# Chriz122/ultralytics_pro

Hardware: AMD Instinct MI355X
Metric: images/sec (whole job = n_gpus x per-GPU bs=32) YOLOv8n 640x640 (forward + Detect decode + NMS) (higher is better)
Workload: dtype bf16

## Files before the change

include/upa.h:

```cpp
#ifndef UPA_H
#define UPA_H
#include <stddef.h>
#include <stdint.h>

#ifdef __cplusplus
extern "C" {
#endif

enum { UPA_F32 = 0, UPA_BF16 = 1, UPA_U8_BGR_HWC = 2  };
enum { UPA_ACT_NONE = 0, UPA_ACT_SILU = 1, UPA_ACT_RELU = 2 };
enum { UPA_OK = 0, UPA_EINVAL = -1, UPA_EUNSUPPORTED = -2, UPA_EWORKSPACE = -3, UPA_ELAUNCH = -4 };

typedef struct upa_opts {
  uint32_t size;
  int32_t conv_big;
  int32_t conv_big_bm;
  int32_t conv_ckt;
  int32_t no_ws, no_pipe, no_1x1, no_c16, no_upcat;
  int32_t pipe_all;
  int32_t pipe_min_tiles;
  int32_t pipe_wgs, c16_wgs;
  int32_t c1_mt, c1_waves, c1_wgs;
  int32_t pair;
  int32_t pair_tile64, pair_tile32;
// ... 2 lines not shown
  int32_t c2f16_waves;
  int32_t c2f32_th;
  int32_t no_branch_tail;
  int32_t branch_tail_bm;
  int32_t stem_wgs, stemf_wgs, stemf_waves, stem_no_mfma;
  int32_t ablate_conv, ablate_pipe, ablate_c1, ablate_stem;
  int32_t c2f64_max_px;
  int32_t conv_ws3;
  int32_t no_group;
  int32_t no_c2f32_up;
  int32_t no_xcd;
  int32_t keys_only;
  int32_t conv_p8;
  int32_t c2f_stream;
  int32_t c2f_stream_rows;
  int32_t no_stack_first;
  int32_t no_epi_stats;
  int32_t nms_stages;
  int32_t nms_first_prefix;
  int32_t detect_stream;
  int32_t detect_stream_rows;
  int32_t no_sppf_front;
  int32_t no_c2f16_down;
} upa_opts;

int upa_version(void);
const char* upa_last_error(void);
size_t upa_opts_size(void);

size_t upa_conv_packed_weight_bytes(int cout, int cin, int k, int dtype);
int upa_pack_conv_weight(const float* w_oihw, int cout, int cin, int k, int dtype, void* out);
int upa_conv2d_bias_act(const void* x, int n, int h, int w, int cin, int ldx,
                        const void* w_packed, const float* bias ,
                        void* y, int cout, int ldy,
                        const void* residual , int ldr,
                        int k, int stride, int pad, int act, int dtype, const upa_opts* opts, void* stream);
typedef struct upa_conv_problem {
  const void* x; int32_t n, h, w, cin, ldx;
  const void* w_packed; const float* bias;
  void* y; int32_t cout, ldy;
  const void* residual; int32_t ldr;
} upa_conv_problem;
int upa_conv2d_bias_act_group(const upa_conv_problem* probs, int count, int k, int stride, int pad, int act, int dtype,
                              const upa_opts* opts, void* stream);

int upa_conv2d_pool2(const void* x, int n, int h, int w, int cin, int ldx, const void* w_packed, const float* bias, void* y, int cout,
// ... 358 lines not shown
```

ultralytics_pro_amd/_lib.py:

```python

from __future__ import annotations

import ctypes as C
import os
from pathlib import Path

import torch

UPA_F32, UPA_BF16, UPA_U8_BGR_HWC = 0, 1, 2
UPA_EINVAL = -1
UPA_EUNSUPPORTED = -2
ACT_NONE, ACT_SILU, ACT_RELU = 0, 1, 2
UPA_PAD_GATHER, UPA_PAD_SCATTER_COPY, UPA_PAD_SCATTER_ADD = 1, 2, 4
MASKS_PLANES, MASKS_OVERLAP = 0, 1
MASK_U8, MASK_F32, MASK_I32 = 0, 1, 2

_PKG = Path(__file__).resolve().parent
LIB_PATH = Path(os.environ.get("UPA_HIP_LIB", _PKG / "libupa_hip.so"))

_vp, _i, _f, _sz = C.c_void_p, C.c_int, C.c_float, C.c_size_t


class Opts(C.Structure):

    _fields_ = [("size", C.c_uint32), ("conv_big", _i), ("conv_big_bm", _i), ("conv_ckt", _i),
                ("no_ws", _i), ("no_pipe", _i), ("no_1x1", _i), ("no_c16", _i), ("no_upcat", _i),
                ("pipe_all", _i), ("pipe_min_tiles", _i), ("pipe_wgs", _i), ("c16_wgs", _i),
                ("c1_mt", _i), ("c1_waves", _i), ("c1_wgs", _i),
                ("pair", _i), ("pair_tile64", _i), ("pair_tile32", _i), ("no_pair_cv2", _i),
                ("c2f", _i), ("c2f16_waves", _i), ("c2f32_th", _i),
                ("no_branch_tail", _i), ("branch_tail_bm", _i),
                ("stem_wgs", _i), ("stemf_wgs", _i), ("stemf_waves", _i), ("stem_no_mfma", _i),
                ("ablate_conv", _i), ("ablate_pipe", _i), ("ablate_c1", _i), ("ablate_stem", _i), ("c2f64_max_px", _i), ("conv_ws3", _i), ("no_group", _i), ("no_c2f32_up", _i), ("no_xcd", _i), ("keys_only", _i), ("conv_p8", _i), ("c2f_stream", _i), ("c2f_stream_rows", _i), ("no_stack_first", _i), ("no_epi_stats", _i), ("nms_stages", _i), ("nms_first_prefix", _i), ("detect_stream", _i), ("detect_stream_rows", _i), ("no_sppf_front", _i), ("no_c2f16_down", _i)]

    def __init__(self, **kw):
        super().__init__()
        self.size = C.sizeof(Opts)
        for k, v in kw.items():
            if k in dict(self._fields_):
                setattr(self, k, int(v))
            else:
                raise AttributeError(f"upa_opts has no field '{k}'")

    def replace(self, **kw) -> "Opts":
        o = Opts()
        C.memmove(C.byref(o), C.byref(self), C.sizeof(Opts))
        for k, v in kw.items():
            setattr(o, k, int(v))
        return o

    _ENV = {"UPA_CONV_BIG": ("conv_big", lambda v: {0: 1, 1: 0, 2: 2}[int(v)]), "UPA_CONV_BIG_BM": ("conv_big_bm", int), "UPA_CONV_WS3": ("conv_ws3", int),
            "UPA_CONV_CKT": ("conv_ckt", int), "UPA_CONV_NO_WS": ("no_ws", lambda v: 1), "UPA_CONV_NO_PIPE": ("no_pipe", lambda v: 1),
            "UPA_CONV_NO_1X1": ("no_1x1", lambda v: 1), "UPA_CONV_NO_C16": ("no_c16", lambda v: 1), "UPA_NO_UPCAT": ("no_upcat", lambda v: 1),
            "UPA_PIPE_ALL": ("pipe_all", lambda v: 1), "UPA_PIPE_MIN_TILES": ("pipe_min_tiles", int), "UPA_PIPE_WGS": ("pipe_wgs", int),
            "UPA_C16_WGS": ("c16_wgs", int), "UPA_C1_MT": ("c1_mt", int), "UPA_C1_WAVES": ("c1_waves", int), "UPA_C1_WGS": ("c1_wgs", int),
            "UPA_NO_PAIR": ("pair", lambda v: {0: 2, 1: 1, 2: 0, 3: 3}[int(v)]), "UPA_PAIR_T64": ("pair_tile64", int),
# ... 245 lines not shown
```

ultralytics_pro_amd/csrc/conv_big.hip:

```cpp
#include <stdlib.h>

#include <mutex>
#include <type_traits>
#include <unordered_map>

#include "common.h"
#include "conv_pipe.h"
UPA_STAMP_DEFINE(conv_big)

template <int KS, int STRIDE, int WM, int WN, int MT, int NT, int TAIL = 0>
__device__ __forceinline__ void conv_big_body(const BigParams& p, const int bid0) {
  static_assert(WM * WN == 8, "8 waves per workgroup");
  static_assert(TAIL == 0 || TAIL == 3 || TAIL == 4 || WN == 1, "a tail needs every channel of a pixel in one wave");
  static_assert(TAIL != 1 || (NT % 2) == 0, "box branch: 64 channels");
  static_assert(TAIL != 3 || (NT % 2) == 0, "the statistics epilogue pairs n-tiles");
  static_assert(TAIL != 4 || ((NT % 2) == 0 && KS == 2 && STRIDE == 1), "the interleaving epilogue: 2 x 2 phase kernels, paired n-tiles");
  constexpr int NTB = WN * NT;
  constexpr int WBUF = 2 * NTB * 1024;
  extern __shared__ __attribute__((aligned(16))) char smem[];
  const int tid = threadIdx.x;
  const int lane = tid & 63;
  const int wave = __builtin_amdgcn_readfirstlane(tid >> 6);
  const int r = lane & 15, g = lane >> 4;
  const int wm = wave / WN, wn = wave % WN;

  const int tilesPerImg = p.tilesX * p.tilesY;
  int bid = p.no_xcd ? bid0 : upa_xcd_tile(bid0, tilesPerImg * p.N);
  const int n = bid / tilesPerImg;
  bid -= n * tilesPerImg;
  const int tyi = bid / p.tilesX;
  const int txi = bid - tyi * p.tilesX;
  const int oy0 = tyi * p.TH, ox0 = txi * p.TW;
  const int iy0 = oy0 * STRIDE - p.pad, ix0 = ox0 * STRIDE - p.pad;
  const int ntb0 = blockIdx.y * NTB;

  const int haloItems = p.IH * p.IWp * 8;
  const int haloPadded = (haloItems + 63) & ~63;
  char* hal = smem;
  char* wbuf = smem + (size_t)haloPadded * 16;

  int pl0[MT], pty[MT], ptx[MT];
#pragma unroll
  for (int i = 0; i < MT; ++i) {
    const int pp = (wm * MT + i) * 16 + r;
    int ty = (int)__umulhi((unsigned)pp, p.magicTW);
    int tx = pp - ty * p.TW;
    if (ty >= p.TH) { ty = p.TH; tx = 0; }
    pty[i] = ty;
    ptx[i] = tx;
    pl0[i] = ty < p.TH ? (ty * STRIDE) * p.IWp + tx : 0;
  }

  f32x4 acc[MT][NT];
#pragma unroll
  for (int i = 0; i < MT; ++i)
#pragma unroll
    for (int j = 0; j < NT; ++j) acc[i][j] = f32x4{0.f, 0.f, 0.f, 0.f};

  constexpr int TAPS = KS * KS;
  const int nChunks = (p.KTT + 1) >> 1;

  auto stage_halo = [&](int c) __attribute__((always_inline)) {
    const int c0 = c * 64;
    for (int base = wave * 64; base < haloPadded; base += 512) {
      const int idx = base + lane;
      const int pix = idx >> 3;
      const int slot = idx & 7;
      const int cg = slot ^ (pix & 7);
      const int py = (int)__umulhi((unsigned)pix, p.magicIW);
      const int qx = pix - py * p.IWp;
      int px = qx;
      if constexpr (STRIDE == 2) px = qx < p.HALF ? 2 * qx : 2 * (qx - p.HALF) + 1;
      const int iy = iy0 + py, ix = ix0 + px;
      const int ch = c0 + cg * 8;
      const char* src = reinterpret_cast<const char*>(g_zero16);
      if (idx < haloItems && px < p.IW && iy >= 0 && iy < p.H && ix >= 0 && ix < p.W && ch < p.Cin)
        src = p.x + ((((size_t)n * p.H + iy) * p.W + ix) * (size_t)p.ldx + ch) * 2;
      lds_dma16(src, hal + base * 16);
    }
  };
  auto stage_w = [&](int c, int tap, int b) __attribute__((always_inline)) {
#pragma unroll
    for (int f0 = 0; f0 < 2 * NTB; f0 += 8) {
      const int f = f0 + wave;
      if (f < 2 * NTB) {
        const int kt = f / NTB, j = f - kt * NTB;
        const int ktg = c * 2 + kt;
        const int nt = ntb0 + j;
        const char* src = reinterpret_cast<const char*>(g_zero16);
        if (ktg < p.KTT && nt < p.NTn) src = p.w + (((size_t)(tap * p.KTT + ktg) * p.NTn + nt) * 64 + lane) * 16;
        lds_dma16(src, wbuf + b * WBUF + f * 1024);
      }
    }
  };

  UPA_STAMP_AT(0);
  UPA_STAMP_HWID();
  stage_halo(0);
  stage_w(0, 0, 0);
  int buf = 0;
  for (int c = 0; c < nChunks; ++c) {
    int kh = 0, kw = 0;
#pragma unroll 1
    for (int tap = 0; tap < TAPS; ++tap) {
      asm volatile("s_waitcnt vmcnt(0)" ::: "memory");
      __syncthreads();
      if (c == 0) UPA_STAMP_AT(1 + tap);
      if (tap + 1 < TAPS) stage_w(c, tap + 1, buf ^ 1);
      const int tapshift = kh * p.IWp + (STRIDE == 2 ? (kw >> 1) + (kw & 1) * p.HALF : kw);
      const char* wb = wbuf + buf * WBUF + (wn * NT) * 1024 + lane * 16;
      int paddr[MT], pswz[MT];
#pragma unroll
      for (int i = 0; i < MT; ++i) {
        const int pl = pl0[i] + tapshift;
        paddr[i] = pl * 128;
        pswz[i] = pl & 7;
      }
#pragma unroll
      for (int kt = 0; kt < 2; ++kt) {
        if constexpr (TAIL == 2) {
          if (kt == 1 && c * 2 + 1 >= p.KTT) break;
        }
        if constexpr (NT <= 6) {
          u32x4 a[NT], b[MT];
#pragma unroll
          for (int j = 0; j < NT; ++j) a[j] = *reinterpret_cast<const u32x4*>(wb + (kt * NTB + j) * 1024);
#pragma unroll
          for (int i = 0; i < MT; ++i) b[i] = *reinterpret_cast<const u32x4*>(hal + paddr[i] + (((kt * 4 + g) ^ pswz[i]) << 4));
#pragma unroll
          for (int i = 0; i < MT; ++i)
#pragma unroll
            for (int j = 0; j < NT; ++j)
              acc[i][j] = __builtin_amdgcn_mfma_f32_16x16x32_bf16(*reinterpret_cast<const bf16x8*>(&a[j]),
                                                                  *reinterpret_cast<const bf16x8*>(&b[i]), acc[i][j], 0, 0, 0);
        } else {
          constexpr int GS = (NT + 1) / 2;
          u32x4 b[MT];
#pragma unroll
          for (int i = 0; i < MT; ++i) b[i] = *reinterpret_cast<const u32x4*>(hal + paddr[i] + (((kt * 4 + g) ^ pswz[i]) << 4));
#pragma unroll
          for (int j0 = 0; j0 < NT; j0 += GS) {
            u32x4 a[GS];
#pragma unroll
            for (int j = 0; j < GS; ++j)
              if (j0 + j < NT) a[j] = *reinterpret_cast<const u32x4*>(wb + (kt * NTB + j0 + j) * 1024);
#pragma unroll
            for (int i = 0; i < MT; ++i)
#pragma unroll
              for (int j = 0; j < GS; ++j)
                if (j0 + j < NT)
                  acc[i][j0 + j] = __builtin_amdgcn_mfma_f32_16x16x32_bf16(*reinterpret_cast<const bf16x8*>(&a[j]),
                                                                           *reinterpret_cast<const bf16x8*>(&b[i]), acc[i][j0 + j], 0, 0, 0);
            __builtin_amdgcn_sched_barrier(0);
          }
        }
      }
      buf ^= 1;
      if (++kw == KS) { kw = 0; ++kh; }
    }
    if (c + 1 < nChunks) {
      __syncthreads();
      stage_halo(c + 1);
      stage_w(c + 1, 0, buf);
    }
  }
  UPA_STAMP_AT(10);

  if constexpr (TAIL == 1 || TAIL == 2) {
    f32x4 bv[NT];
#pragma unroll
    for (int j = 0; j < NT; ++j) bv[j] = *reinterpret_cast<const f32x4*>(p.bias + j * 16 + g * 4);
    f32x4 acc2[MT][NT];
#pragma unroll
    for (int i = 0; i < MT; ++i)
#pragma unroll
      for (int j = 0; j < NT; ++j) acc2[i][j] = f32x4{0.f, 0.f, 0.f, 0.f};
#pragma unroll
    for (int s2 = 0; s2 < NT / 2; ++s2) {
      u32x4 hb[MT];
#pragma unroll
      for (int i = 0; i < MT; ++i) {
        float v0[4], v1[4];
#pragma unroll
        for (int q = 0; q < 4; ++q) {
          v0[q] = act_rcp<UPA_ACT_SILU>(acc[i][2 * s2][q] + bv[2 * s2][q]);
          v1[q] = act_rcp<UPA_ACT_SILU>(acc[i][2 * s2 + 1][q] + bv[2 * s2 + 1][q]);
// ... 201 lines not shown
            const u32x2 rv = *reinterpret_cast<const u32x2*>(rrow + cb * 2);
            v[0] += __uint_as_float(rv[0] << 16); v[1] += __uint_as_float(rv[0] & 0xFFFF0000u);
            v[2] += __uint_as_float(rv[1] << 16); v[3] += __uint_as_float(rv[1] & 0xFFFF0000u);
          }
          *reinterpret_cast<u32x2*>(yrow + cb * 2) = u32x2{pack_bf16x2(v[0], v[1]), pack_bf16x2(v[2], v[3])};
        }
      }
    }
  };
  if (p.act == UPA_ACT_SILU) epilogue(std::integral_constant<int, UPA_ACT_SILU>{});
  else if (p.act == UPA_ACT_RELU) epilogue(std::integral_constant<int, UPA_ACT_RELU>{});
  else epilogue(std::integral_constant<int, UPA_ACT_NONE>{});
  UPA_STAMP_AT(11);
#ifdef UPA_STAMP
  asm volatile("s_waitcnt vmcnt(0)" ::: "memory");
  UPA_STAMP_AT(12);
#endif
}

template <int KS, int STRIDE, int WM, int WN, int MT, int NT, int TAIL = 0>
__global__ __launch_bounds__(512, 4) void conv_big_kernel(const BigParams p) {
  conv_big_body<KS, STRIDE, WM, WN, MT, NT, TAIL>(p, (int)blockIdx.x);
}

template <int KS, int STRIDE, int WM, int WN, int MT, int NT, int TAIL = 0>
__global__ __launch_bounds__(512, 4) void conv_big_pair_kernel(const BigParams p0, const BigParams p1, const int split) {
  if ((int)blockIdx.x < split) conv_big_body<KS, STRIDE, WM, WN, MT, NT, TAIL>(p0, (int)blockIdx.x);
  else conv_big_body<KS, STRIDE, WM, WN, MT, NT, TAIL>(p1, (int)blockIdx.x - split);
}
template <int KS, int STRIDE, int WM, int WN, int MT, int NT, int TAIL = 0>
__global__ __launch_bounds__(512, 4) void conv_big_tri_kernel(const BigParams p0, const BigParams p1, const BigParams p2, const int s0,
                                                              const int s1) {
  if ((int)blockIdx.x < s0) conv_big_body<KS, STRIDE, WM, WN, MT, NT, TAIL>(p0, (int)blockIdx.x);
  else if ((int)blockIdx.x < s1) conv_big_body<KS, STRIDE, WM, WN, MT, NT, TAIL>(p1, (int)blockIdx.x - s0);
  else conv_big_body<KS, STRIDE, WM, WN, MT, NT, TAIL>(p2, (int)blockIdx.x - s1);
}

template <int KS_, int STRIDE_, int WM_, int WN_, int MT_, int NT_, int TAIL_>
struct BigCfg {
  static constexpr int NTB = WN_ * NT_;
  __device__ static __forceinline__ void run(const BigParams& p, int bid) { conv_big_body<KS_, STRIDE_, WM_, WN_, MT_, NT_, TAIL_>(p, bid); }
};
template <class CA, class CB>
__global__ __launch_bounds__(512, 4) void conv_big_mix_kernel(const BigParams a0, const BigParams a1, const BigParams b0, const BigParams b1,
                                                              const int s0, const int s1, const int s2) {
  const int b = (int)blockIdx.x;
  if (b < s0) CA::run(a0, b);
  else if (b < s1) CA::run(a1, b - s0);
  else if (b < s2) CB::run(b0, b - s1);
  else CB::run(b1, b - s2);
}

namespace {
void big_halo_geometry(BigParams& p, bool tight = false) {
  p.IH = (p.TH - 1) * p.stride + p.KS;
  p.IW = (p.TW - 1) * p.stride + p.KS;
  p.HALF = p.stride == 2 ? (p.IW + 1) / 2 : 0;
  const int minp = p.stride == 2 ? 2 * p.HALF : p.IW;
  p.IWp = tight ? minp : upa_lds_pick_pitch(minp, p.TW, p.TH * p.TW, p.stride);
  p.magicTW = (unsigned)((0x100000000ULL + p.TW - 1) / p.TW);
  p.magicIW = (unsigned)((0x100000000ULL + p.IWp - 1) / p.IWp);
}
size_t big_halo_bytes(const BigParams& p) { return (((size_t)p.IH * p.IWp * 8 + 63) & ~(size_t)63) * 16; }

bool big_pick_tile(BigParams& p, int bm, int ntb, size_t lds_cap) {
  struct Pick { int th, tw, tight; };
  static std::mutex mu;
  static std::unordered_map<unsigned long long, Pick> memo;
  const unsigned long long key = ((unsigned long long)p.OH << 48) ^ ((unsigned long long)p.OW << 32) ^ ((unsigned long long)bm << 20) ^
                                 ((unsigned long long)ntb << 12) ^ ((unsigned long long)(lds_cap >> 9) << 3) ^ ((unsigned long long)p.KS << 56) ^ (p.KS == 3 ? 4u : 0u) ^
                                 (p.stride == 2 ? 2u : 0u);
  {
    std::lock_guard<std::mutex> lk(mu);
// ... 21 lines not shown
        big_halo_geometry(p, tight != 0);
        const size_t lds = big_halo_bytes(p) + 2 * (size_t)(2 * ntb * 1024) + 256;
        if (lds > lds_cap) continue;
        const long tiles = (long)cdiv(p.OW, tw) * cdiv(p.OH, th);
        const long cost = tiles * 65536 + (long)p.IH * p.IWp;
        if (best < 0 || cost < best) { best = cost; bth = th; btw = tw; btight = tight != 0; }
        break;
      }
    }
  }
  p.TH = bth; p.TW = btw;
  if (best >= 0) big_halo_geometry(p, btight);
  {
    std::lock_guard<std::mutex> lk(mu);
    memo[key] = Pick{best >= 0 ? bth : 0, btw, btight ? 1 : 0};
  }
  return best >= 0;
}

template <int KS, int STRIDE, int WM, int WN, int MT, int NT, int TAIL = 0>
int big_launch_inst(const BigParams& p, size_t lds, hipStream_t s) {
  constexpr int NTB = WN * NT;
  const dim3 grid((unsigned)((long)p.tilesX * p.tilesY * p.N), (unsigned)cdiv(p.NTn, NTB));
  auto kern = conv_big_kernel<KS, STRIDE, WM, WN, MT, NT, TAIL>;
  if (hipError_t e = upa_full_lds<conv_big_kernel<KS, STRIDE, WM, WN, MT, NT, TAIL>>(); e != hipSuccess) {
    upa_set_error("conv_big: cannot raise LDS limit: %s", hipGetErrorString(e));
    return UPA_ELAUNCH;
  }
  hipLaunchKernelGGL(kern, grid, dim3(512), lds, s, p);
  UPA_LAUNCH_CHECK();
  return UPA_OK;
}

template <int KS, int STRIDE, int WM, int WN, int MT, int NT, int TAIL = 0>
int big_launch_pair_inst(const BigParams& p0, const BigParams& p1, size_t lds, hipStream_t s) {
  constexpr int NTB = WN * NT;
  const long t0 = (long)p0.tilesX * p0.tilesY * p0.N, t1 = (long)p1.tilesX * p1.tilesY * p1.N;
  if (cdiv(p0.NTn, NTB) != cdiv(p1.NTn, NTB) || t0 + t1 >= (1L << 31)) return UPA_EUNSUPPORTED;
  const dim3 grid((unsigned)(t0 + t1), (unsigned)cdiv(p0.NTn, NTB));
  if (hipError_t e = upa_full_lds<conv_big_pair_kernel<KS, STRIDE, WM, WN, MT, NT, TAIL>>(); e != hipSuccess) {
    upa_set_error("conv_big: cannot raise LDS limit: %s", hipGetErrorString(e));
    return UPA_ELAUNCH;
  }
  hipLaunchKernelGGL((conv_big_pair_kernel<KS, STRIDE, WM, WN, MT, NT, TAIL>), grid, dim3(512), lds, s, p0, p1, (int)t0);
  UPA_LAUNCH_CHECK();
  return UPA_OK;
}

template <int KS, int STRIDE, int WM, int WN, int MT, int NT, int TAIL = 0>
int big_launch_tri_inst(const BigParams& p0, const BigParams& p1, const BigParams& p2, size_t lds, hipStream_t s) {
  constexpr int NTB = WN * NT;
  const long t0 = (long)p0.tilesX * p0.tilesY * p0.N, t1 = (long)p1.tilesX * p1.tilesY * p1.N, t2 = (long)p2.tilesX * p2.tilesY * p2.N;
  if (cdiv(p0.NTn, NTB) != cdiv(p1.NTn, NTB) || cdiv(p0.NTn, NTB) != cdiv(p2.NTn, NTB) || t0 + t1 + t2 >= (1L << 31)) return UPA_EUNSUPPORTED;
  const dim3 grid((unsigned)(t0 + t1 + t2), (unsigned)cdiv(p0.NTn, NTB));
  if (hipError_t e = upa_full_lds<conv_big_tri_kernel<KS, STRIDE, WM, WN, MT, NT, TAIL>>(); e != hipSuccess) {
    upa_set_error("conv_big: cannot raise LDS limit: %s", hipGetErrorString(e));
    return UPA_ELAUNCH;
  }
  hipLaunchKernelGGL((conv_big_tri_kernel<KS, STRIDE, WM, WN, MT, NT, TAIL>), grid, dim3(512), lds, s, p0, p1, p2, (int)t0, (int)(t0 + t1));
  UPA_LAUNCH_CHECK();
  return UPA_OK;
}

template <class CA, class CB>
int big_launch_mix(const BigParams* pa, int na, const BigParams* pb, int nb, size_t lds, hipStream_t s) {
  long t[4] = {0, 0, 0, 0};
  for (int i = 0; i < na; ++i) { t[i] = (long)pa[i].tilesX * pa[i].tilesY * pa[i].N; if (pa[i].NTn > CA::NTB) return UPA_EUNSUPPORTED; }
  for (int i = 0; i < nb; ++i) { t[2 + i] = (long)pb[i].tilesX * pb[i].tilesY * pb[i].N; if (pb[i].NTn > CB::NTB) return UPA_EUNSUPPORTED; }
  const long tot = t[0] + t[1] + t[2] + t[3];
  if (tot >= (1L << 31)) return UPA_EUNSUPPORTED;
  if (hipError_t e = upa_full_lds<conv_big_mix_kernel<CA, CB>>(); e != hipSuccess) {
    upa_set_error("conv_big: cannot raise LDS limit: %s", hipGetErrorString(e));
    return UPA_ELAUNCH;
  }
  hipLaunchKernelGGL((conv_big_mix_kernel<CA, CB>), dim3((unsigned)tot), dim3(512), lds, s, pa[0], pa[na > 1 ? 1 : 0], pb[0], pb[nb > 1 ? 1 : 0],
                     (int)t[0], (int)(t[0] + t[1]), (int)(t[0] + t[1] + t[2]));
  UPA_LAUNCH_CHECK();
  return UPA_OK;
}

template <int WM, int WN, int MT, int NT>
int big_launch_ks(const BigParams& p, size_t lds, hipStream_t s) {
  if (p.KS == 1) return big_launch_inst<1, 1, WM, WN, MT, NT>(p, lds, s);
  if (p.KS == 2) return big_launch_inst<2, 1, WM, WN, MT, NT>(p, lds, s);
  if (p.stride == 2) return big_launch_inst<3, 2, WM, WN, MT, NT>(p, lds, s);
  return big_launch_inst<3, 1, WM, WN, MT, NT>(p, lds, s);
}
}

extern "C" size_t upa_tail_packed_weight_bytes(int cout, int cin) {
  return (size_t)cdiv(cin, 32) * cdiv(cout, 16) * 1024;
}

// ... 207 lines not shown
  p.NTn = (p.Cout + 15) / 16;
  ntb = p.NTn <= 4 ? 4 : (p.NTn <= 6 ? 6 : 8);
  if (p.NTn == 5 && p.KS == 3 && p.stride == 1) ntb = 5;
  if (p.NTn == 9 && p.KS == 3 && p.stride == 1) ntb = 9;
  if (force_ntb == 5 && p.NTn <= 5 && p.KS == 3 && p.stride == 1) ntb = 5;
  const long px = (long)p.N * p.OH * p.OW;
  if (ntb == 8 && p.NTn % 4 == 0 && (px + 127) / 128 * cdiv(p.NTn, 8) < upa_num_cus()) ntb = 4;
  const int cols = cdiv(p.NTn, ntb);
  bm = 256;
  if ((px + 255) / 256 * cols < upa_num_cus()) bm = 128;
  if (const int f = UPA_OPT(opts, conv_big_bm); f == 128 || f == 256 || (f == 512 && p.KS == 3 && p.stride == 1 && (ntb == 4 || ntb == 5))) bm = f;
  if (query_only) return UPA_OK;
  if (p.KS == 1) {
    p.N = 1; p.H = 1; p.W = (int)px; p.OH = 1; p.OW = (int)px;
    p.TH = 1; p.TW = bm;
    big_halo_geometry(p, true);
  } else if (!big_pick_tile(p, bm, ntb, 80 * 1024 - 512) && !big_pick_tile(p, bm, ntb, 160 * 1024)) {
    return UPA_EUNSUPPORTED;
  }
  p.tilesX = cdiv(p.OW, p.TW);
  p.tilesY = cdiv(p.OH, p.TH);
  lds = big_halo_bytes(p) + 2 * (size_t)(2 * ntb * 1024) + 256;
  if (lds > 160 * 1024) return UPA_EUNSUPPORTED;
  return UPA_OK;
}
template <int WM, int WN, int MT, int NT>
int big_launch_ks_stats(const BigParams& p, size_t lds, hipStream_t s) {
  if (p.KS == 1) return big_launch_inst<1, 1, WM, WN, MT, NT, 3>(p, lds, s);
  if (p.KS != 3) return UPA_EUNSUPPORTED;
  if (p.stride == 2) return big_launch_inst<3, 2, WM, WN, MT, NT, 3>(p, lds, s);
  return big_launch_inst<3, 1, WM, WN, MT, NT, 3>(p, lds, s);
}
int big_dispatch_stats(const BigParams& p, int ntb, int bm, size_t lds, hipStream_t s) {
  if (bm != 128 && bm != 256) return UPA_EUNSUPPORTED;
  if (ntb == 8) return bm == 256 ? big_launch_ks_stats<4, 2, 4, 4>(p, lds, s) : big_launch_ks_stats<4, 2, 2, 4>(p, lds, s);
  if (ntb == 4) return bm == 256 ? big_launch_ks_stats<8, 1, 2, 4>(p, lds, s) : big_launch_ks_stats<4, 2, 2, 2>(p, lds, s);
  return UPA_EUNSUPPORTED;
}
int big_dispatch(const BigParams& p, int ntb, int bm, size_t lds, hipStream_t s) {
  if (bm == 512) return ntb == 5 ? big_launch_inst<3, 1, 8, 1, 4, 5>(p, lds, s) : big_launch_inst<3, 1, 8, 1, 4, 4>(p, lds, s);
  if (ntb == 5) return bm == 256 ? big_launch_inst<3, 1, 8, 1, 2, 5>(p, lds, s) : big_launch_inst<3, 1, 8, 1, 1, 5>(p, lds, s);
  if (ntb == 9) return bm == 256 ? big_launch_inst<3, 1, 8, 1, 2, 9>(p, lds, s) : big_launch_inst<3, 1, 8, 1, 1, 9>(p, lds, s);
  if (ntb == 8) return bm == 256 ? big_launch_ks<4, 2, 4, 4>(p, lds, s) : big_launch_ks<4, 2, 2, 4>(p, lds, s);
  if (ntb == 6) return bm == 256 ? big_launch_ks<4, 2, 4, 3>(p, lds, s) : big_launch_ks<4, 2, 2, 3>(p, lds, s);
  return bm == 256 ? big_launch_ks<8, 1, 2, 4>(p, lds, s) : big_launch_ks<4, 2, 2, 2>(p, lds, s);
}
}

int upa_conv_big_launch(BigParams p, int query_only, int* variant, void* stream, const upa_opts* opts) {
  p.no_xcd = UPA_OPT(opts, no_xcd);
  int ntb = 0, bm = 0;
  size_t lds = 0;
  const int rc = big_prepare(p, ntb, bm, lds, opts, query_only != 0);
  if (variant) *variant = (1 << 23) | (ntb << 4) | (bm >> 7);
  if (query_only || rc != UPA_OK) return rc;
  return big_dispatch(p, ntb, bm, lds, (hipStream_t)stream);
}

int upa_conv_big_launch_interleave(BigParams p, void* stream, const upa_opts* opts) {
  p.no_xcd = UPA_OPT(opts, no_xcd);
  if (p.KS != 2 || p.stride != 1 || p.act != UPA_ACT_NONE || p.bias || p.il_c % 8 != 0 || p.Cout != 4 * p.il_c) return UPA_EUNSUPPORTED;
  int ntb = 0, bm = 0;
  size_t lds = 0;
  if (const int rc = big_prepare(p, ntb, bm, lds, opts, false); rc != UPA_OK) return rc;
  if (ntb != 8 || (bm != 128 && bm != 256)) return UPA_EUNSUPPORTED;
  hipStream_t s = (hipStream_t)stream;
  return bm == 256 ? big_launch_inst<2, 1, 4, 2, 4, 4, 4>(p, lds, s) : big_launch_inst<2, 1, 4, 2, 2, 4, 4>(p, lds, s);
}

int upa_conv_big_launch_stats(BigParams p, int* rows, long max_rows, void* stream, const upa_opts* opts) {
  p.no_xcd = UPA_OPT(opts, no_xcd);
  if (!p.stats || p.res || p.act != UPA_ACT_NONE) return UPA_EUNSUPPORTED;
  int ntb = 0, bm = 0;
  size_t lds = 0;
  if (const int rc = big_prepare(p, ntb, bm, lds, opts, false); rc != UPA_OK) return rc;
  if ((ntb != 8 && ntb != 4) || (bm != 128 && bm != 256)) return UPA_EUNSUPPORTED;
  const long nrows = (long)p.tilesX * p.tilesY * p.N;
  if (nrows > max_rows) return UPA_EUNSUPPORTED;
  p.stats_ld = p.NTn * 16;
  *rows = (int)nrows;
  return big_dispatch_stats(p, ntb, bm, lds, (hipStream_t)stream);
}

int upa_conv_big_launch_group(const BigParams* probs, int count, int* consumed, void* stream, const upa_opts* opts) {
  *consumed = 0;
  if (count < 2) return UPA_EUNSUPPORTED;
  const int grouping = UPA_OPT(opts, no_group);
  if (grouping == 1) return UPA_EUNSUPPORTED;
  if (count >= 4) {
    BigParams q[4];
    int nt4[4], bm4[4];
    size_t l4[4];
    bool ok = true;
    for (int i = 0; i < 4 && ok; ++i) {
      q[i] = probs[i];
      ok = q[i].KS == 3 && q[i].stride == 1 && big_prepare(q[i], nt4[i], bm4[i], l4[i], opts, false) == UPA_OK && bm4[i] == 128;
    }
    if (ok && nt4[0] == 4 && nt4[1] == 4 && nt4[2] == 5 && nt4[3] == 5) {
      size_t l = l4[0];
      for (int i = 1; i < 4; ++i) l = l4[i] > l ? l4[i] : l;
      const bool sw0 = q[1].Cin > q[0].Cin, sw1 = q[3].Cin > q[2].Cin;
      const BigParams a[2] = {sw1 ? q[3] : q[2], sw1 ? q[2] : q[3]}, b[2] = {sw0 ? q[1] : q[0], sw0 ? q[0] : q[1]};
      const int rc = big_launch_mix<BigCfg<3, 1, 8, 1, 1, 5, 0>, BigCfg<3, 1, 4, 2, 2, 2, 0>>(a, 2, b, 2, l, (hipStream_t)stream);
      if (rc == UPA_OK) { *consumed = 4; return UPA_OK; }
      if (rc != UPA_EUNSUPPORTED) return rc;
    }
  }
  BigParams p[3];
  int ntb[3], bm[3];
  size_t lds[3];
  const int m = count >= 3 && grouping == 2 ? 3 : 2;
  for (int i = 0; i < m; ++i) {
    p[i] = probs[i];
    if (p[i].KS != 3 || p[i].stride != 1) return UPA_EUNSUPPORTED;
    if (const int rc = big_prepare(p[i], ntb[i], bm[i], lds[i], opts, false); rc != UPA_OK) return rc;
  }
  hipStream_t s = (hipStream_t)stream;
  auto ok_ntb = [](int v) { return v == 4 || v == 5; };
  if (m == 3 && ntb[0] == ntb[1] && ntb[0] == ntb[2] && ok_ntb(ntb[0]) && bm[1] == 128 && bm[2] == 128) {
    int rc = UPA_OK;
    if (bm[0] != 128) {
      upa_opts o;
      memset(&o, 0, sizeof(o));
      if (opts) memcpy(&o, opts, opts->size < sizeof(o) ? opts->size : sizeof(o));
      o.size = sizeof(o);
      o.conv_big_bm = 128;
      p[0] = probs[0];
      rc = big_prepare(p[0], ntb[0], bm[0], lds[0], &o, false);
    }
    if (rc == UPA_OK && bm[0] == 128 && ntb[0] == ntb[1]) {
      const size_t l3 = lds[0] > lds[1] ? (lds[0] > lds[2] ? lds[0] : lds[2]) : (lds[1] > lds[2] ? lds[1] : lds[2]);
      rc = ntb[0] == 4 ? big_launch_tri_inst<3, 1, 4, 2, 2, 2>(p[0], p[1], p[2], l3, s) : big_launch_tri_inst<3, 1, 8, 1, 1, 5>(p[0], p[1], p[2], l3, s);
      if (rc == UPA_OK) { *consumed = 3; return UPA_OK; }
      if (rc != UPA_EUNSUPPORTED) return rc;
    }
    p[0] = probs[0];
    if (const int rc2 = big_prepare(p[0], ntb[0], bm[0], lds[0], opts, false); rc2 != UPA_OK) return rc2;
  }
  if (ok_ntb(ntb[0]) && ok_ntb(ntb[1]) && bm[0] == bm[1] && (bm[0] == 128 || bm[0] == 256)) {
    if (ntb[0] != ntb[1]) {
      const int lo = ntb[0] < ntb[1] ? 0 : 1;
      p[lo] = probs[lo];
      int bmf = 0;
      if (const int rc = big_prepare(p[lo], ntb[lo], bmf, lds[lo], opts, false, 5); rc != UPA_OK) return rc;
      if (bmf != bm[1 - lo] || ntb[lo] != 5) return UPA_EUNSUPPORTED;
    }
    const size_t l2 = lds[0] > lds[1] ? lds[0] : lds[1];
    int rc;
    if (bm[0] == 128) rc = ntb[0] == 4 ? big_launch_pair_inst<3, 1, 4, 2, 2, 2>(p[0], p[1], l2, s) : big_launch_pair_inst<3, 1, 8, 1, 1, 5>(p[0], p[1], l2, s);
    else rc = ntb[0] == 4 ? big_launch_pair_inst<3, 1, 8, 1, 2, 4>(p[0], p[1], l2, s) : big_launch_pair_inst<3, 1, 8, 1, 2, 5>(p[0], p[1], l2, s);
    if (rc == UPA_OK) { *consumed = 2; return UPA_OK; }
    if (rc != UPA_EUNSUPPORTED) return rc;
  }
  return UPA_EUNSUPPORTED;
}
```

ultralytics_pro_amd/csrc/conv_pipe.h:

```cpp
#pragma once
struct ConvShape {
  int n, h, w, cin, ldx, cout, ldy, ldr, k, stride, pad, act, dtype;
};
struct PipeParams {
  const char* x;
  char* y;
  const char* res;
  const char* w;
  const float* bias;
  int N, H, W, Cin, ldx, Cout, ldy, ldr;
  int KTT, NTn, nt0;
  int tilesX, tilesY, numTiles;
  int act;
  int pool;
#ifdef UPA_ABLATE
  int ablate;
#endif
};
bool upa_conv_pipe_eligible(const ConvShape& s, const upa_opts* opts);
int upa_conv_pipe_launch(PipeParams p, int query_only, int* variant, void* stream, const upa_opts* opts);

#include "detect_epi.h"
struct C1Params {
  const char* x;
// ... 14 lines not shown
  const char* up;
  int upKT, up_ld, upH, upW;
  unsigned upMagicW, upMagicH;
};
bool upa_conv1x1_eligible(const ConvShape& s, const upa_opts* opts);
int upa_conv1x1_launch(C1Params p, int n_pixels, int query_only, int* variant, void* stream, const upa_opts* opts);
int upa_conv1x1_launch_stats(C1Params p, int n_pixels, int* rows, long max_rows, void* stream, const upa_opts* opts);

struct BigParams {
  const char* x;
  char* y;
  const char* res;
  const char* w;
  const float* bias;
  int N, H, W, Cin, ldx, OH, OW, Cout, ldy, ldr;
  int KS, stride, pad;
  int TH, TW, tilesX, tilesY, IH, IW;
  int IWp;
  int HALF;
  int KTT, NTn;
  int act;
  unsigned magicTW, magicIW;
  int no_xcd;
  const char* tw;
  const float* tb;
  DetectEpi de;
  float* stats;
  int stats_ld;
  int il_h, il_w, il_c;
};
bool upa_conv_big_eligible(const ConvShape& s, const upa_opts* opts);
int upa_conv_big_launch(BigParams p, int query_only, int* variant, void* stream, const upa_opts* opts);
int upa_conv_big_launch_stats(BigParams p, int* rows, long max_rows, void* stream, const upa_opts* opts);
int upa_conv_big_launch_interleave(BigParams p, void* stream, const upa_opts* opts);
int upa_conv_big_launch_group(const BigParams* probs, int count, int* consumed, void* stream, const upa_opts* opts);

bool upa_conv_big_pick_tile(BigParams& p, int bm, int ntb, size_t lds_cap);

bool upa_conv_p8_eligible(const ConvShape& s, const upa_opts* opts);
int upa_conv_p8_launch(BigParams p, int query_only, int* variant, void* stream, const upa_opts* opts);

bool upa_conv_ws3_eligible(const ConvShape& s, const upa_opts* opts);
int upa_conv_ws3_launch(BigParams p, int query_only, int* variant, void* stream, const upa_opts* opts);
int upa_conv_ws3_launch_stats(BigParams p, int* rows, long max_rows, void* stream, const upa_opts* opts);

struct PairParams {
// ... 17 lines not shown
```

Before: 61990.

## Stage several input-channel chunks of halo per sync in conv_big

Adds a grouped form of the big implicit-GEMM convolution that stages G channel chunks of the input halo into LDS at once, so there are fewer barrier-separated halo reloads per tile. For 1x1 kernels it also keeps the weights for every chunk in the group resident, which drops the per-tap barrier. For other kernel sizes it prefetches the next chunk's first-tap weights across the chunk boundary. G is chosen automatically from the LDS budget and workgroup count, or forced by a new conv_big_group option. The cost is more LDS per workgroup, which can lower occupancy.

```diff
diff --git a/include/upa.h b/include/upa.h
--- a/include/upa.h
+++ b/include/upa.h
@@ -48,6 +48,7 @@
   int32_t detect_stream_rows;
   int32_t no_sppf_front;
   int32_t no_c2f16_down;
+  int32_t conv_big_group;
 } upa_opts;
 
 int upa_version(void);
diff --git a/ultralytics_pro_amd/_lib.py b/ultralytics_pro_amd/_lib.py
--- a/ultralytics_pro_amd/_lib.py
+++ b/ultralytics_pro_amd/_lib.py
@@ -31,7 +31,7 @@
                 ("c2f", _i), ("c2f16_waves", _i), ("c2f32_th", _i),
                 ("no_branch_tail", _i), ("branch_tail_bm", _i),
                 ("stem_wgs", _i), ("stemf_wgs", _i), ("stemf_waves", _i), ("stem_no_mfma", _i),
-                ("ablate_conv", _i), ("ablate_pipe", _i), ("ablate_c1", _i), ("ablate_stem", _i), ("c2f64_max_px", _i), ("conv_ws3", _i), ("no_group", _i), ("no_c2f32_up", _i), ("no_xcd", _i), ("keys_only", _i), ("conv_p8", _i), ("c2f_stream", _i), ("c2f_stream_rows", _i), ("no_stack_first", _i), ("no_epi_stats", _i), ("nms_stages", _i), ("nms_first_prefix", _i), ("detect_stream", _i), ("detect_stream_rows", _i), ("no_sppf_front", _i), ("no_c2f16_down", _i)]
+                ("ablate_conv", _i), ("ablate_pipe", _i), ("ablate_c1", _i), ("ablate_stem", _i), ("c2f64_max_px", _i), ("conv_ws3", _i), ("no_group", _i), ("no_c2f32_up", _i), ("no_xcd", _i), ("keys_only", _i), ("conv_p8", _i), ("c2f_stream", _i), ("c2f_stream_rows", _i), ("no_stack_first", _i), ("no_epi_stats", _i), ("nms_stages", _i), ("nms_first_prefix", _i), ("detect_stream", _i), ("detect_stream_rows", _i), ("no_sppf_front", _i), ("no_c2f16_down", _i), ("conv_big_group", _i)]
 
     def __init__(self, **kw):
         super().__init__()
diff --git a/ultralytics_pro_amd/csrc/conv_big.hip b/ultralytics_pro_amd/csrc/conv_big.hip
--- a/ultralytics_pro_amd/csrc/conv_big.hip
+++ b/ultralytics_pro_amd/csrc/conv_big.hip
@@ -8,7 +8,8 @@
 #include "conv_pipe.h"
 UPA_STAMP_DEFINE(conv_big)
 
-template <int KS, int STRIDE, int WM, int WN, int MT, int NT, int TAIL = 0>
+constexpr bool big_groups(int tail, int mt, int nt) { return tail == 0 && nt <= 6 && mt * nt <= 16; }
+template <int KS, int STRIDE, int WM, int WN, int MT, int NT, int TAIL = 0, bool GRP = false>
 __device__ __forceinline__ void conv_big_body(const BigParams& p, const int bid0) {
   static_assert(WM * WN == 8, "8 waves per workgroup");
   static_assert(TAIL == 0 || TAIL == 3 || TAIL == 4 || WN == 1, "a tail needs every channel of a pixel in one wave");
@@ -36,8 +37,12 @@
 
   const int haloItems = p.IH * p.IWp * 8;
   const int haloPadded = (haloItems + 63) & ~63;
+  static_assert(!GRP || big_groups(TAIL, MT, NT), "no grouped form of this variant");
+  const int G = !GRP ? 1 : (p.G > 1 ? p.G : 1);
+  const int haloBytes = haloPadded * 16;
+  const bool resident = KS == 1 && G > 1;
   char* hal = smem;
-  char* wbuf = smem + (size_t)haloPadded * 16;
+  char* wbuf = smem + (size_t)G * haloBytes;
 
   int pl0[MT], pty[MT], ptx[MT];
 #pragma unroll
@@ -60,8 +65,9 @@
   constexpr int TAPS = KS * KS;
   const int nChunks = (p.KTT + 1) >> 1;
 
-  auto stage_halo = [&](int c) __attribute__((always_inline)) {
+  auto stage_halo = [&](int c, int hb) __attribute__((always_inline)) {
     const int c0 = c * 64;
+    char* dst = hal + hb * haloBytes;
     for (int base = wave * 64; base < haloPadded; base += 512) {
       const int idx = base + lane;
       const int pix = idx >> 3;
@@ -76,7 +82,7 @@
       const char* src = reinterpret_cast<const char*>(g_zero16);
       if (idx < haloItems && px < p.IW && iy >= 0 && iy < p.H && ix >= 0 && ix < p.W && ch < p.Cin)
         src = p.x + ((((size_t)n * p.H + iy) * p.W + ix) * (size_t)p.ldx + ch) * 2;
-      lds_dma16(src, hal + base * 16);
+      lds_dma16(src, dst + base * 16);
     }
   };
   auto stage_w = [&](int c, int tap, int b) __attribute__((always_inline)) {
@@ -94,74 +100,119 @@
     }
   };
 
+  auto multiply = [&](int c, const char* wb, const int (&paddr)[MT], const int (&pswz)[MT]) __attribute__((always_inline)) {
+#pragma unroll
+    for (int kt = 0; kt < 2; ++kt) {
+      if constexpr (TAIL == 2) {
+        if (kt == 1 && c * 2 + 1 >= p.KTT) break;
+      }
+      if constexpr (NT <= 6) {
+        u32x4 a[NT], b[MT];
+#pragma unroll
+        for (int j = 0; j < NT; ++j) a[j] = *reinterpret_cast<const u32x4*>(wb + (kt * NTB + j) * 1024);
+#pragma unroll
+        for (int i = 0; i < MT; ++i) b[i] = *reinterpret_cast<const u32x4*>(hal + paddr[i] + (((kt * 4 + g) ^ pswz[i]) << 4));
+#pragma unroll
+        for (int i = 0; i < MT; ++i)
+#pragma unroll
+          for (int j = 0; j < NT; ++j)
+            acc[i][j] = __builtin_amdgcn_mfma_f32_16x16x32_bf16(*reinterpret_cast<const bf16x8*>(&a[j]),
+                                                                *reinterpret_cast<const bf16x8*>(&b[i]), acc[i][j], 0, 0, 0);
+      } else {
+        constexpr int GS = (NT + 1) / 2;
+        u32x4 b[MT];
+#pragma unroll
+        for (int i = 0; i < MT; ++i) b[i] = *reinterpret_cast<const u32x4*>(hal + paddr[i] + (((kt * 4 + g) ^ pswz[i]) << 4));
+#pragma unroll
+        for (int j0 = 0; j0 < NT; j0 += GS) {
+          u32x4 a[GS];
+#pragma unroll
+          for (int j = 0; j < GS; ++j)
+            if (j0 + j < NT) a[j] = *reinterpret_cast<const u32x4*>(wb + (kt * NTB + j0 + j) * 1024);
+#pragma unroll
+          for (int i = 0; i < MT; ++i)
+#pragma unroll
+            for (int j = 0; j < GS; ++j)
+              if (j0 + j < NT)
+                acc[i][j0 + j] = __builtin_amdgcn_mfma_f32_16x16x32_bf16(*reinterpret_cast<const bf16x8*>(&a[j]),
+                                                                         *reinterpret_cast<const bf16x8*>(&b[i]), acc[i][j0 + j], 0, 0, 0);
+          __builtin_amdgcn_sched_barrier(0);
+        }
+      }
+    }
+  };
   UPA_STAMP_AT(0);
   UPA_STAMP_HWID();
-  stage_halo(0);
-  stage_w(0, 0, 0);
   int buf = 0;
-  for (int c = 0; c < nChunks; ++c) {
-    int kh = 0, kw = 0;
+  if constexpr (!GRP) {
+    stage_halo(0, 0);
+    stage_w(0, 0, 0);
+    for (int c = 0; c < nChunks; ++c) {
+      int kh = 0, kw = 0;
 #pragma unroll 1
-    for (int tap = 0; tap < TAPS; ++tap) {
-      asm volatile("s_waitcnt vmcnt(0)" ::: "memory");
-      __syncthreads();
-      if (c == 0) UPA_STAMP_AT(1 + tap);
-      if (tap + 1 < TAPS) stage_w(c, tap + 1, buf ^ 1);
-      const int tapshift = kh * p.IWp + (STRIDE == 2 ? (kw >> 1) + (kw & 1) * p.HALF : kw);
-      const char* wb = wbuf + buf * WBUF + (wn * NT) * 1024 + lane * 16;
-      int paddr[MT], pswz[MT];
-#pragma unroll
-      for (int i = 0; i < MT; ++i) {
-        const int pl = pl0[i] + tapshift;
-        paddr[i] = pl * 128;
-        pswz[i] = pl & 7;
-      }
-#pragma unroll
-      for (int kt = 0; kt < 2; ++kt) {
-        if constexpr (TAIL == 2) {
-          if (kt == 1 && c * 2 + 1 >= p.KTT) break;
+      for (int tap = 0; tap < TAPS; ++tap) {
+        asm volatile("s_waitcnt vmcnt(0)" ::: "memory");
+        __syncthreads();
+        if (c == 0) UPA_STAMP_AT(1 + tap);
+        if (tap + 1 < TAPS) stage_w(c, tap + 1, buf ^ 1);
+        const int tapshift = kh * p.IWp + (STRIDE == 2 ? (kw >> 1) + (kw & 1) * p.HALF : kw);
+        const char* wb = wbuf + buf * WBUF + (wn * NT) * 1024 + lane * 16;
+        int paddr[MT], pswz[MT];
+#pragma unroll
+        for (int i = 0; i < MT; ++i) {
+          const int pl = pl0[i] + tapshift;
+          paddr[i] = pl * 128;
+          pswz[i] = pl & 7;
         }
-        if constexpr (NT <= 6) {
-          u32x4 a[NT], b[MT];
-#pragma unroll
-          for (int j = 0; j < NT; ++j) a[j] = *reinterpret_cast<const u32x4*>(wb + (kt * NTB + j) * 1024);
-#pragma unroll
-          for (int i = 0; i < MT; ++i) b[i] = *reinterpret_cast<const u32x4*>(hal + paddr[i] + (((kt * 4 + g) ^ pswz[i]) << 4));
-#pragma unroll
-          for (int i = 0; i < MT; ++i)
-#pragma unroll
-            for (int j = 0; j < NT; ++j)
-              acc[i][j] = __builtin_amdgcn_mfma_f32_16x16x32_bf16(*reinterpret_cast<const bf16x8*>(&a[j]),
-                                                                  *reinterpret_cast<const bf16x8*>(&b[i]), acc[i][j], 0, 0, 0);
-        } else {
-          constexpr int GS = (NT + 1) / 2;
-          u32x4 b[MT];
-#pragma unroll
-          for (int i = 0; i < MT; ++i) b[i] = *reinterpret_cast<const u32x4*>(hal + paddr[i] + (((kt * 4 + g) ^ pswz[i]) << 4));
-#pragma unroll
-          for (int j0 = 0; j0 < NT; j0 += GS) {
-            u32x4 a[GS];
-#pragma unroll
-            for (int j = 0; j < GS; ++j)
-              if (j0 + j < NT) a[j] = *reinterpret_cast<const u32x4*>(wb + (kt * NTB + j0 + j) * 1024);
-#pragma unroll
-            for (int i = 0; i < MT; ++i)
-#pragma unroll
-              for (int j = 0; j < GS; ++j)
-                if (j0 + j < NT)
-                  acc[i][j0 + j] = __builtin_amdgcn_mfma_f32_16x16x32_bf16(*reinterpret_cast<const bf16x8*>(&a[j]),
-                                                                           *reinterpret_cast<const bf16x8*>(&b[i]), acc[i][j0 + j], 0, 0, 0);
-            __builtin_amdgcn_sched_barrier(0);
+        multiply(c, wb, paddr, pswz);
+        buf ^= 1;
+        if (++kw == KS) { kw = 0; ++kh; }
+      }
+      if (c + 1 < nChunks) {
+        __syncthreads();
+        stage_halo(c + 1, 0);
+        stage_w(c + 1, 0, buf);
+      }
+    }
+  } else {
+    for (int c0 = 0; c0 < nChunks; c0 += G) {
+      const int cEnd = c0 + G < nChunks ? c0 + G : nChunks;
+      if (c0 > 0) __syncthreads();
+#pragma unroll 1
+      for (int c = c0; c < cEnd; ++c) stage_halo(c, c - c0);
+      if (resident) {
+#pragma unroll 1
+        for (int c = c0; c < cEnd; ++c) stage_w(c, 0, c - c0);
+      } else {
+        stage_w(c0, 0, buf);
+      }
+      int hoff = 0;
+#pragma unroll 1
+      for (int c = c0; c < cEnd; ++c, hoff += haloBytes) {
+        int kh = 0, kw = 0;
+#pragma unroll 1
+        for (int tap = 0; tap < TAPS; ++tap) {
+          if (!resident || c == c0) {
+            asm volatile("s_waitcnt vmcnt(0)" ::: "memory");
+            __syncthreads();
           }
+          if (c == 0) UPA_STAMP_AT(1 + tap);
+          if (tap + 1 < TAPS) stage_w(c, tap + 1, buf ^ 1);
+          else if (KS != 1 && c + 1 < cEnd) stage_w(c + 1, 0, buf ^ 1);
+          const int tapshift = kh * p.IWp + (STRIDE == 2 ? (kw >> 1) + (kw & 1) * p.HALF : kw);
+          const char* wb = wbuf + (resident ? c - c0 : buf) * WBUF + (wn * NT) * 1024 + lane * 16;
+          int paddr[MT], pswz[MT];
+#pragma unroll
+          for (int i = 0; i < MT; ++i) {
+            const int pl = pl0[i] + tapshift;
+            paddr[i] = pl * 128 + hoff;
+            pswz[i] = pl & 7;
+          }
+          multiply(c, wb, paddr, pswz);
+          buf ^= 1;
+          if (++kw == KS) { kw = 0; ++kh; }
         }
       }
-      buf ^= 1;
-      if (++kw == KS) { kw = 0; ++kh; }
-    }
-    if (c + 1 < nChunks) {
-      __syncthreads();
-      stage_halo(c + 1);
-      stage_w(c + 1, 0, buf);
     }
   }
   UPA_STAMP_AT(10);
@@ -409,11 +460,20 @@
 __global__ __launch_bounds__(512, 4) void conv_big_kernel(const BigParams p) {
   conv_big_body<KS, STRIDE, WM, WN, MT, NT, TAIL>(p, (int)blockIdx.x);
 }
+template <int KS, int STRIDE, int WM, int WN, int MT, int NT, int TAIL = 0>
+__global__ __launch_bounds__(512, 4) void conv_big_grouped_kernel(const BigParams p) {
+  conv_big_body<KS, STRIDE, WM, WN, MT, NT, TAIL, true>(p, (int)blockIdx.x);
+}
 
 template <int KS, int STRIDE, int WM, int WN, int MT, int NT, int TAIL = 0>
 __global__ __launch_bounds__(512, 4) void conv_big_pair_kernel(const BigParams p0, const BigParams p1, const int split) {
   if ((int)blockIdx.x < split) conv_big_body<KS, STRIDE, WM, WN, MT, NT, TAIL>(p0, (int)blockIdx.x);
   else conv_big_body<KS, STRIDE, WM, WN, MT, NT, TAIL>(p1, (int)blockIdx.x - split);
+}
+template <int KS, int STRIDE, int WM, int WN, int MT, int NT, int TAIL = 0>
+__global__ __launch_bounds__(512, 4) void conv_big_pair_grouped_kernel(const BigParams p0, const BigParams p1, const int split) {
+  if ((int)blockIdx.x < split) conv_big_body<KS, STRIDE, WM, WN, MT, NT, TAIL, true>(p0, (int)blockIdx.x);
+  else conv_big_body<KS, STRIDE, WM, WN, MT, NT, TAIL, true>(p1, (int)blockIdx.x - split);
 }
 template <int KS, int STRIDE, int WM, int WN, int MT, int NT, int TAIL = 0>
 __global__ __launch_bounds__(512, 4) void conv_big_tri_kernel(const BigParams p0, const BigParams p1, const BigParams p2, const int s0,
@@ -422,20 +482,38 @@
   else if ((int)blockIdx.x < s1) conv_big_body<KS, STRIDE, WM, WN, MT, NT, TAIL>(p1, (int)blockIdx.x - s0);
   else conv_big_body<KS, STRIDE, WM, WN, MT, NT, TAIL>(p2, (int)blockIdx.x - s1);
 }
+template <int KS, int STRIDE, int WM, int WN, int MT, int NT, int TAIL = 0>
+__global__ __launch_bounds__(512, 4) void conv_big_tri_grouped_kernel(const BigParams p0, const BigParams p1, const BigParams p2, const int s0,
+                                                                      const int s1) {
+  if ((int)blockIdx.x < s0) conv_big_body<KS, STRIDE, WM, WN, MT, NT, TAIL, true>(p0, (int)blockIdx.x);
+  else if ((int)blockIdx.x < s1) conv_big_body<KS, STRIDE, WM, WN, MT, NT, TAIL, true>(p1, (int)blockIdx.x - s0);
+  else conv_big_body<KS, STRIDE, WM, WN, MT, NT, TAIL, true>(p2, (int)blockIdx.x - s1);
+}
 
 template <int KS_, int STRIDE_, int WM_, int WN_, int MT_, int NT_, int TAIL_>
 struct BigCfg {
   static constexpr int NTB = WN_ * NT_;
-  __device__ static __forceinline__ void run(const BigParams& p, int bid) { conv_big_body<KS_, STRIDE_, WM_, WN_, MT_, NT_, TAIL_>(p, bid); }
+  static constexpr bool GROUPS = big_groups(TAIL_, MT_, NT_);
+  template <bool GRP>
+  __device__ static __forceinline__ void run(const BigParams& p, int bid) { conv_big_body<KS_, STRIDE_, WM_, WN_, MT_, NT_, TAIL_, GRP && GROUPS>(p, bid); }
 };
 template <class CA, class CB>
 __global__ __launch_bounds__(512, 4) void conv_big_mix_kernel(const BigParams a0, const BigParams a1, const BigParams b0, const BigParams b1,
                                                               const int s0, const int s1, const int s2) {
   const int b = (int)blockIdx.x;
-  if (b < s0) CA::run(a0, b);
-  else if (b < s1) CA::run(a1, b - s0);
-  else if (b < s2) CB::run(b0, b - s1);
-  else CB::run(b1, b - s2);
+  if (b < s0) CA::template run<false>(a0, b);
+  else if (b < s1) CA::template run<false>(a1, b - s0);
+  else if (b < s2) CB::template run<false>(b0, b - s1);
+  else CB::template run<false>(b1, b - s2);
+}
+template <class CA, class CB>
+__global__ __launch_bounds__(512, 4) void conv_big_mix_grouped_kernel(const BigParams a0, const BigParams a1, const BigParams b0, const BigParams b1,
+                                                                      const int s0, const int s1, const int s2) {
+  const int b = (int)blockIdx.x;
+  if (b < s0) CA::template run<true>(a0, b);
+  else if (b < s1) CA::template run<true>(a1, b - s0);
+  else if (b < s2) CB::template run<true>(b0, b - s1);
+  else CB::template run<true>(b1, b - s2);
 }
 
 namespace {
@@ -503,6 +581,17 @@
 int big_launch_inst(const BigParams& p, size_t lds, hipStream_t s) {
   constexpr int NTB = WN * NT;
   const dim3 grid((unsigned)((long)p.tilesX * p.tilesY * p.N), (unsigned)cdiv(p.NTn, NTB));
+  if constexpr (big_groups(TAIL, MT, NT)) {
+    if (p.G > 1) {
+      if (hipError_t e = upa_full_lds<conv_big_grouped_kernel<KS, STRIDE, WM, WN, MT, NT, TAIL>>(); e != hipSuccess) {
+        upa_set_error("conv_big: cannot raise LDS limit: %s", hipGetErrorString(e));
+        return UPA_ELAUNCH;
+      }
+      hipLaunchKernelGGL((conv_big_grouped_kernel<KS, STRIDE, WM, WN, MT, NT, TAIL>), grid, dim3(512), lds, s, p);
+      UPA_LAUNCH_CHECK();
+      return UPA_OK;
+    }
+  }
   auto kern = conv_big_kernel<KS, STRIDE, WM, WN, MT, NT, TAIL>;
   if (hipError_t e = upa_full_lds<conv_big_kernel<KS, STRIDE, WM, WN, MT, NT, TAIL>>(); e != hipSuccess) {
     upa_set_error("conv_big: cannot raise LDS limit: %s", hipGetErrorString(e));
@@ -519,6 +608,17 @@
   const long t0 = (long)p0.tilesX * p0.tilesY * p0.N, t1 = (long)p1.tilesX * p1.tilesY * p1.N;
   if (cdiv(p0.NTn, NTB) != cdiv(p1.NTn, NTB) || t0 + t1 >= (1L << 31)) return UPA_EUNSUPPORTED;
   const dim3 grid((unsigned)(t0 + t1), (unsigned)cdiv(p0.NTn, NTB));
+  if constexpr (big_groups(TAIL, MT, NT)) {
+    if (p0.G > 1 || p1.G > 1) {
+      if (hipError_t e = upa_full_lds<conv_big_pair_grouped_kernel<KS, STRIDE, WM, WN, MT, NT, TAIL>>(); e != hipSuccess) {
+        upa_set_error("conv_big: cannot raise LDS limit: %s", hipGetErrorString(e));
+        return UPA_ELAUNCH;
+      }
+      hipLaunchKernelGGL((conv_big_pair_grouped_kernel<KS, STRIDE, WM, WN, MT, NT, TAIL>), grid, dim3(512), lds, s, p0, p1, (int)t0);
+      UPA_LAUNCH_CHECK();
+      return UPA_OK;
+    }
+  }
   if (hipError_t e = upa_full_lds<conv_big_pair_kernel<KS, STRIDE, WM, WN, MT, NT, TAIL>>(); e != hipSuccess) {
     upa_set_error("conv_big: cannot raise LDS limit: %s", hipGetErrorString(e));
     return UPA_ELAUNCH;
@@ -534,6 +634,17 @@
   const long t0 = (long)p0.tilesX * p0.tilesY * p0.N, t1 = (long)p1.tilesX * p1.tilesY * p1.N, t2 = (long)p2.tilesX * p2.tilesY * p2.N;
   if (cdiv(p0.NTn, NTB) != cdiv(p1.NTn, NTB) || cdiv(p0.NTn, NTB) != cdiv(p2.NTn, NTB) || t0 + t1 + t2 >= (1L << 31)) return UPA_EUNSUPPORTED;
   const dim3 grid((unsigned)(t0 + t1 + t2), (unsigned)cdiv(p0.NTn, NTB));
+  if constexpr (big_groups(TAIL, MT, NT)) {
+    if (p0.G > 1 || p1.G > 1 || p2.G > 1) {
+      if (hipError_t e = upa_full_lds<conv_big_tri_grouped_kernel<KS, STRIDE, WM, WN, MT, NT, TAIL>>(); e != hipSuccess) {
+        upa_set_error("conv_big: cannot raise LDS limit: %s", hipGetErrorString(e));
+        return UPA_ELAUNCH;
+      }
+      hipLaunchKernelGGL((conv_big_tri_grouped_kernel<KS, STRIDE, WM, WN, MT, NT, TAIL>), grid, dim3(512), lds, s, p0, p1, p2, (int)t0, (int)(t0 + t1));
+      UPA_LAUNCH_CHECK();
+      return UPA_OK;
+    }
+  }
   if (hipError_t e = upa_full_lds<conv_big_tri_kernel<KS, STRIDE, WM, WN, MT, NT, TAIL>>(); e != hipSuccess) {
     upa_set_error("conv_big: cannot raise LDS limit: %s", hipGetErrorString(e));
     return UPA_ELAUNCH;
@@ -550,6 +661,21 @@
   for (int i = 0; i < nb; ++i) { t[2 + i] = (long)pb[i].tilesX * pb[i].tilesY * pb[i].N; if (pb[i].NTn > CB::NTB) return UPA_EUNSUPPORTED; }
   const long tot = t[0] + t[1] + t[2] + t[3];
   if (tot >= (1L << 31)) return UPA_EUNSUPPORTED;
+  if constexpr (CA::GROUPS || CB::GROUPS) {
+    bool grouped = false;
+    for (int i = 0; i < na; ++i) grouped = grouped || pa[i].G > 1;
+    for (int i = 0; i < nb; ++i) grouped = grouped || pb[i].G > 1;
+    if (grouped) {
+      if (hipError_t e = upa_full_lds<conv_big_mix_grouped_kernel<CA, CB>>(); e != hipSuccess) {
+        upa_set_error("conv_big: cannot raise LDS limit: %s", hipGetErrorString(e));
+        return UPA_ELAUNCH;
+      }
+      hipLaunchKernelGGL((conv_big_mix_grouped_kernel<CA, CB>), dim3((unsigned)tot), dim3(512), lds, s, pa[0], pa[na > 1 ? 1 : 0], pb[0], pb[nb > 1 ? 1 : 0],
+                         (int)t[0], (int)(t[0] + t[1]), (int)(t[0] + t[1] + t[2]));
+      UPA_LAUNCH_CHECK();
+      return UPA_OK;
+    }
+  }
   if (hipError_t e = upa_full_lds<conv_big_mix_kernel<CA, CB>>(); e != hipSuccess) {
     upa_set_error("conv_big: cannot raise LDS limit: %s", hipGetErrorString(e));
     return UPA_ELAUNCH;
@@ -803,6 +929,40 @@
   p.tilesY = cdiv(p.OH, p.TH);
   lds = big_halo_bytes(p) + 2 * (size_t)(2 * ntb * 1024) + 256;
   if (lds > 160 * 1024) return UPA_EUNSUPPORTED;
+  p.G = 1;
+  return UPA_OK;
+}
+size_t big_group_lds(const BigParams& p, int ntb, int g) {
+  return (size_t)g * big_halo_bytes(p) + (size_t)(p.KS == 1 && g > 2 ? g : 2) * (2 * ntb * 1024) + 256;
+}
+int big_pick_group(BigParams& p, int ntb, int bm, long wgs, size_t& lds, const upa_opts* opts) {
+  const int nChunks = (p.KTT + 1) / 2;
+  const int force = UPA_OPT(opts, conv_big_group);
+  const size_t whole = 160 * 1024, half = 80 * 1024 - 512;
+  p.G = 1;
+  const int wn = (ntb == 8 || ntb == 6 || (ntb == 4 && bm == 128)) ? 2 : 1;
+  if (force == 0 || force == 1 || nChunks == 1 || !big_groups(0, bm * wn / 128, ntb / wn)) return UPA_OK;
+  if (force >= 2) {
+    const int g = force < nChunks ? force : nChunks;
+    if (big_group_lds(p, ntb, g) > whole) {
+      upa_set_error("conv_big: a group of %d chunks needs %zu bytes of LDS", g, big_group_lds(p, ntb, g));
+      return UPA_EINVAL;
+    }
+    p.G = g;
+  } else {
+    const size_t cap = (lds > half || wgs <= upa_num_cus()) ? whole : half;
+    for (int g = nChunks; g > 1; --g)
+      if (big_group_lds(p, ntb, g) <= cap) { p.G = g; break; }
+  }
+  lds = big_group_lds(p, ntb, p.G);
+  return UPA_OK;
+}
+long big_wgs(const BigParams& p, int ntb) { return (long)p.tilesX * p.tilesY * p.N * cdiv(p.NTn, ntb); }
+int big_pick_groups(BigParams* p, const int* ntb, const int* bm, size_t* lds, int m, const upa_opts* opts) {
+  long wgs = 0;
+  for (int i = 0; i < m; ++i) wgs += big_wgs(p[i], ntb[i]);
+  for (int i = 0; i < m; ++i)
+    if (const int rc = big_pick_group(p[i], ntb[i], bm[i], wgs, lds[i], opts); rc != UPA_OK) return rc;
   return UPA_OK;
 }
 template <int WM, int WN, int MT, int NT>
@@ -835,6 +995,7 @@
   const int rc = big_prepare(p, ntb, bm, lds, opts, query_only != 0);
   if (variant) *variant = (1 << 23) | (ntb << 4) | (bm >> 7);
   if (query_only || rc != UPA_OK) return rc;
+  if (const int rg = big_pick_group(p, ntb, bm, big_wgs(p, ntb), lds, opts); rg != UPA_OK) return rg;
   return big_dispatch(p, ntb, bm, lds, (hipStream_t)stream);
 }
 
@@ -878,6 +1039,7 @@
       ok = q[i].KS == 3 && q[i].stride == 1 && big_prepare(q[i], nt4[i], bm4[i], l4[i], opts, false) == UPA_OK && bm4[i] == 128;
     }
     if (ok && nt4[0] == 4 && nt4[1] == 4 && nt4[2] == 5 && nt4[3] == 5) {
+      if (const int rc = big_pick_groups(q, nt4, bm4, l4, 4, opts); rc != UPA_OK) return rc;
       size_t l = l4[0];
       for (int i = 1; i < 4; ++i) l = l4[i] > l ? l4[i] : l;
       const bool sw0 = q[1].Cin > q[0].Cin, sw1 = q[3].Cin > q[2].Cin;
@@ -909,6 +1071,7 @@
       p[0] = probs[0];
       rc = big_prepare(p[0], ntb[0], bm[0], lds[0], &o, false);
     }
+    if (rc == UPA_OK && bm[0] == 128 && ntb[0] == ntb[1]) rc = big_pick_groups(p, ntb, bm, lds, 3, opts);
     if (rc == UPA_OK && bm[0] == 128 && ntb[0] == ntb[1]) {
       const size_t l3 = lds[0] > lds[1] ? (lds[0] > lds[2] ? lds[0] : lds[2]) : (lds[1] > lds[2] ? lds[1] : lds[2]);
       rc = ntb[0] == 4 ? big_launch_tri_inst<3, 1, 4, 2, 2, 2>(p[0], p[1], p[2], l3, s) : big_launch_tri_inst<3, 1, 8, 1, 1, 5>(p[0], p[1], p[2], l3, s);
@@ -917,6 +1080,7 @@
     }
     p[0] = probs[0];
     if (const int rc2 = big_prepare(p[0], ntb[0], bm[0], lds[0], opts, false); rc2 != UPA_OK) return rc2;
+    if (const int rc2 = big_prepare(p[1] = probs[1], ntb[1], bm[1], lds[1], opts, false); rc2 != UPA_OK) return rc2;
   }
   if (ok_ntb(ntb[0]) && ok_ntb(ntb[1]) && bm[0] == bm[1] && (bm[0] == 128 || bm[0] == 256)) {
     if (ntb[0] != ntb[1]) {
@@ -926,6 +1090,7 @@
       if (const int rc = big_prepare(p[lo], ntb[lo], bmf, lds[lo], opts, false, 5); rc != UPA_OK) return rc;
       if (bmf != bm[1 - lo] || ntb[lo] != 5) return UPA_EUNSUPPORTED;
     }
+    if (const int rg = big_pick_groups(p, ntb, bm, lds, 2, opts); rg != UPA_OK) return rg;
     const size_t l2 = lds[0] > lds[1] ? lds[0] : lds[1];
     int rc;
     if (bm[0] == 128) rc = ntb[0] == 4 ? big_launch_pair_inst<3, 1, 4, 2, 2, 2>(p[0], p[1], l2, s) : big_launch_pair_inst<3, 1, 8, 1, 1, 5>(p[0], p[1], l2, s);
diff --git a/ultralytics_pro_amd/csrc/conv_pipe.h b/ultralytics_pro_amd/csrc/conv_pipe.h
--- a/ultralytics_pro_amd/csrc/conv_pipe.h
+++ b/ultralytics_pro_amd/csrc/conv_pipe.h
@@ -60,6 +60,7 @@
   int act;
   unsigned magicTW, magicIW;
   int no_xcd;
+  int G;
   const char* tw;
   const float* tb;
   DetectEpi de;
```

Result: no change. 61980 (median of 2 runs) (-0.0%).
